# mstksg/tensor-ops

Hardware: AMD Instinct MI355X
Metric: gradTOp steps/sec (ffLayer MNIST 784->256->10) + gmul TFLOP/s vs roofline (higher is better)
Workload: dtype f32

## Files before the change

tensor-ops_amd/csrc/gemm_small.hip:

```cpp
#include "common.hpp"

#include <type_traits>

namespace to {

typedef float f32x16 __attribute__((ext_vector_type(16)));

template <class S>
struct SmallArgsT {
  const S* A;
  const S* B;
  S* C;
  const S* Cin;
  int M, N, K;
  long a_sm, a_sk, b_sk, b_sn, c_sm;
  long a_sb, b_sb, c_sb;
  int a_vec, b_vec;
  unsigned a_bytes, b_bytes;
  int tiles_n;
  int tiles_m;
  int tile_order;
  int kper;
  S alpha, beta;
  const S* bias;
// ... 17 lines not shown
};

#ifdef TOPS_AB_KNOBS
#define SM_STAMP(i) do { if (stamp_on) g.dbg[i] = wall_clock64(); } while (0)
#else
#define SM_STAMP(i) do { } while (0)
#endif


template <class G>
__device__ __forceinline__ void tile_of(const G& g, int bid, int& tile_m, int& tile_n) {
  if (g.tile_order) {
    const int T = g.tiles_m * g.tiles_n, x = bid & 7, q = T >> 3, r = T & 7;
    bid = (x < r ? x * (q + 1) : r * (q + 1) + (x - r) * q) + (bid >> 3);
  }
  if (g.tile_order == 2) {
    tile_n = bid / g.tiles_m;
    tile_m = bid - tile_n * g.tiles_m;
  } else {
    tile_m = bid / g.tiles_n;
    tile_n = bid - tile_m * g.tiles_n;
  }
}

__device__ __forceinline__ float tanh_s(float x) { return tanhf(x); }
__device__ __forceinline__ double tanh_s(double x) { return tanh(x); }
__device__ __forceinline__ float exp_s(float x) { return expf(x); }
__device__ __forceinline__ double exp_s(double x) { return exp(x); }
__device__ __forceinline__ float log_s(float x) { return logf(x); }
__device__ __forceinline__ double log_s(double x) { return log(x); }
__device__ __forceinline__ float max_s(float a, float b) { return fmaxf(a, b); }
__device__ __forceinline__ double max_s(double a, double b) { return fmax(a, b); }

template <class S, int AMODE, int BMODE, int NW, int TS, int ONESHOT = 0, bool EXT = false, int PARTS = 0, bool STAG = false>
__device__ __forceinline__ void gemm_small_body(const SmallArgsT<S>& g, const int bid, const long bz, S* ext_lds = nullptr,
                                                const int tid_in = -1) {
  constexpr int ES = (int)sizeof(S);
  static_assert(ES == 4 || TS == 16, "the fp64 matrix instruction is 16x16x4");
  constexpr int KG = (TS == 32) ? 2 : 4;
  constexpr int NR = (TS == 32) ? 16 : 4;
  constexpr int CK = 4 * KG;
  typedef S accv __attribute__((ext_vector_type(NR)));
  S (*red)[NR][64];
  S (*rsum)[64];
  S* dzs;
  if constexpr (EXT) {
    red = reinterpret_cast<S (*)[NR][64]>(ext_lds);
    rsum = reinterpret_cast<S (*)[64]>(ext_lds + NW * NR * 64);
    dzs = ext_lds + NW * NR * 64 + NW * 64;
  } else {
    __shared__ S red_s[NW][NR][64];
    __shared__ S rsum_s[NW][64];
    __shared__ S dzs_s[TS == 16 ? 16 * 17 : 1];
    red = red_s;
    rsum = rsum_s;
    dzs = dzs_s;
  }
  const int tid = tid_in >= 0 ? tid_in : (int)threadIdx.x, lane = tid & 63, wave = tid >> 6;
  const int l31 = lane & (TS - 1), half = lane / TS;
#ifdef TOPS_AB_KNOBS
  const bool stamp_on = g.dbg && bid == 0 && tid == 0;
#endif
  SM_STAMP(0);
  int tile_m, tile_n;
  tile_of(g, bid, tile_m, tile_n);
  const long m = (long)tile_m * TS + l31, n = (long)tile_n * TS + l31;
// ... 204 lines not shown
    }
  }
#pragma unroll
  for (int r = 0; r < NR; ++r) red[wave][r][lane] = acc[r];
  rsum[wave][lane] = asum;
  SM_STAMP(4);
  __syncthreads();
  SM_STAMP(5);
  if (g.rowsum && tile_n == 0 && wave == 0 && lane < TS) {
    S v = S(0);
#pragma unroll
    for (int w = 0; w < NW; ++w)
#pragma unroll
      for (int q = 0; q < KG; ++q) v += rsum[w][lane + q * TS];
    const long row = (long)tile_m * TS + lane;
    if (row < g.M) g.rowsum[bz * g.M + row] = g.rowsum_acc ? g.rowsum_in[bz * g.M + row] + g.rowsum_alpha * v : v;
  }
#pragma unroll
  for (int i = 0; i < NRW; ++i) {
    const int r = wave + i * NW;
    if (r >= NR) break;
    S v = S(0);
#pragma unroll
    for (int w = 0; w < NW; ++w) v += red[w][r][lane];
    const int lrow = (TS == 32) ? (r & 3) + 8 * (r >> 2) + 4 * half : row16(half, r);
    const long row = (long)tile_m * TS + lrow;
    const long col = (long)tile_n * TS + l31;
    if constexpr (TS == 16) {
      if (g.loss_rows) {
        const bool valid = row < g.M && col < g.N;
        v = v * g.alpha + pf_bias;
        const S t = valid ? g.target[row * g.c_sm + col] : S(0);
        auto sum16 = [](S x) {
#pragma unroll
          for (int off = 8; off > 0; off >>= 1) x += __shfl_xor(x, off, 64);
          return x;
        };
        S out, l;
        if (g.loss_rows == 1) {
          S mx = valid ? v : S(-INFINITY);
#pragma unroll
          for (int off = 8; off > 0; off >>= 1) mx = max_s(mx, __shfl_xor(mx, off, 64));
          const S e = valid ? exp_s(v - mx) : S(0);
          const S se = sum16(e), sy = sum16(t);
          const S pr = e / se;
          out = pr * sy - t;
          l = valid ? -t * log_s(pr) : S(0);
        } else {
          const S sg = S(1) / (S(1) + exp_s(-v));
          const S e = t - sg;
          out = S(-2) * e * sg * (S(1) - sg);
          l = valid ? e * e : S(0);
        }
        if (valid) Cb[row * g.c_sm + col] = out;
        if (g.tail_out) dzs[lrow * 17 + l31] = valid ? out : S(0);
        if (g.loss_out) {
          l = sum16(l);
          if (l31 == 0 && row < g.M) g.loss_out[row] = l;
        }
        continue;
      }
    }
    if (row < g.M && col < g.N) {
      v *= g.alpha;
      if (Ci) v += g.beta * pf_ci[i];
      v += pf_bias;
      if (g.act == 1) v = S(1) / (S(1) + exp_s(-v));
      else if (g.act == 2) v = tanh_s(v);
      if (Hd) {
        const S h = pf_hd[i];
        v *= g.dact_kind ? S(1) - h * h : h * (S(1) - h);
      }
      Cb[row * g.c_sm + col] = v;
    }
  }
// ... 12 lines not shown
#pragma unroll
      for (int st = 0; st < 4; ++st) {
        if (4 * st < g.N) {
          const S a = dzs[l15 * 17 + 4 * st + kg];
#pragma unroll
          for (int u = 0; u < 2; ++u) {
            if constexpr (ES == 8) acc2[u] = __builtin_amdgcn_mfma_f64_16x16x4f64(a, tl_bw[u][st], acc2[u], 0, 0, 0);
            else acc2[u] = __builtin_amdgcn_mfma_f32_16x16x4f32(a, tl_bw[u][st], acc2[u], 0, 0, 0);
          }
        }
      }
#pragma unroll
      for (int u = 0; u < 2; ++u) {
        const int t = wave + u * NW;
        const long col = (long)t * 16 + l15;
#pragma unroll
        for (int r = 0; r < 4; ++r) {
          const long row = (long)tile_m * 16 + row16(kg, r);
          if (t < ntiles && row < g.M && col < g.tail_n)
            g.tail_out[row * g.tail_n + col] = acc2[u][r] * tl_hv[u][r] * (S(1) - tl_hv[u][r]);
        }
      }
      SM_STAMP(7);
    }
  }
#ifdef TOPS_AB_KNOBS
  if (stamp_on) { __builtin_amdgcn_s_waitcnt(0); SM_STAMP(8); }
#endif
}

template <class S, int AMODE, int BMODE, int NW, int TS, int ONESHOT = 0>
__global__ __launch_bounds__(NW * 64) void gemm_small_kernel(SmallArgsT<S> g) {
  gemm_small_body<S, AMODE, BMODE, NW, TS, ONESHOT>(g, (int)blockIdx.x, (long)blockIdx.z);
}

template <class S, int A1, int B1, int NW1, int TS1, int OS1, int A2, int B2, int NW2, int TS2, int OS2, int P1 = 0, bool STAG1 = false>
__global__ __launch_bounds__((NW1 > NW2 ? NW1 : NW2) * 64) void gemm_small_pair_kernel(SmallArgsT<S> g1,
                                                                                         SmallArgsT<S> g2, int n1) {
  if ((int)blockIdx.x < n1) {
    if (NW1 < NW2 && (int)(threadIdx.x >> 6) >= NW1) return;
    gemm_small_body<S, A1, B1, NW1, TS1, OS1, false, P1, STAG1>(g1, (int)blockIdx.x, 0);
  } else {
    if (NW2 < NW1 && (int)(threadIdx.x >> 6) >= NW2) return;
    gemm_small_body<S, A2, B2, NW2, TS2, OS2>(g2, (int)blockIdx.x - n1, 0);
  }
}

struct ChainSync {
  unsigned* ctr;
  int* status;
  long long timeout;
  int dev;
};

__device__ __forceinline__ bool chain_barrier(const ChainSync& cs, int which, unsigned epoch) {
  __shared__ int ok;
  if (cs.dev == 1) {
    __syncthreads();
    return true;
  }
  if (cs.dev != 2) __builtin_amdgcn_fence(__ATOMIC_RELEASE, "agent");
  if (threadIdx.x == 0) ok = 1;
  __syncthreads();
  unsigned* flags = cs.ctr + which * 256;
  if (threadIdx.x == 0) __hip_atomic_store(flags + blockIdx.x, epoch, __ATOMIC_RELEASE, __HIP_MEMORY_SCOPE_AGENT);
  if (threadIdx.x < gridDim.x) {
// ... 433 lines not shown
}

template <class S>
static void launch_small_t(const GemmProblem& p, hipStream_t s) {
  constexpr bool F64 = sizeof(S) == 8;
  SmallArgsT<S> g;
  const SmallPlan c = plan_small<S>(p, g);
#ifdef TOPS_AB_KNOBS
  if (g.loss_rows) g.dbg = small_stamps(2);
#endif
  const int amode = c.amode, bmode = c.bmode;
  if constexpr (F64) {
    if (c.f64_t32) {
      const int tiles_m = (int)((p.M + 31) / 32);
      dim3 grid(tiles_m * g.tiles_n, 1, (unsigned)p.batch), block(c.nw * 64);
#define TOPS_F64_T32(AM, BM)                                                                              \
  switch (c.nw * 10 + c.os) {                                                                             \
    case 22: launch_k((gemm_small_f64_t32_kernel<AM, BM, 2, 2>), grid, block, 0, s, g); break;  \
    case 42: launch_k((gemm_small_f64_t32_kernel<AM, BM, 4, 2>), grid, block, 0, s, g); break;  \
    default: launch_k((gemm_small_f64_t32_kernel<AM, BM, 8, 1>), grid, block, 0, s, g); break;  \
  }
      switch (amode * 2 + bmode) {
        case 0: TOPS_F64_T32(0, 0) break;
        case 1: TOPS_F64_T32(0, 1) break;
        case 2: TOPS_F64_T32(1, 0) break;
        default: TOPS_F64_T32(1, 1) break;
      }
#undef TOPS_F64_T32
      TO_HIP(hipGetLastError());
      count_launch();
      return;
    }
  }
  if (c.os == 8 && c.nw == 16) {
    if constexpr (!F64) launch_nw<S, 16, 32, 8>(g, p, amode, bmode, s);
  } else if (c.os == 8) {
    launch_nw<S, 8, 16, 8>(g, p, amode, bmode, s);
  } else if (c.ts == 16) {
    switch (c.nw) {
      case 1: launch_nw<S, 1, 16>(g, p, amode, bmode, s); break;
      case 2: launch_nw<S, 2, 16>(g, p, amode, bmode, s); break;
      case 4: launch_nw<S, 4, 16>(g, p, amode, bmode, s); break;
      default: launch_nw<S, 8, 16>(g, p, amode, bmode, s); break;
    }
  } else {
    if constexpr (!F64) {
      switch (c.nw) {
        case 1: launch_nw<S, 1, 32>(g, p, amode, bmode, s); break;
        case 2: launch_nw<S, 2, 32>(g, p, amode, bmode, s); break;
        case 4: launch_nw<S, 4, 32>(g, p, amode, bmode, s); break;
        default: launch_nw<S, 8, 32>(g, p, amode, bmode, s); break;
      }
    }
  }
  TO_HIP(hipGetLastError());
  count_launch();
}

static int* g_chain_status = nullptr;

bool launch_gemm_small_chain(const GemmProblem& pa, const GemmProblem& pb, const GemmProblem& pc1, const GemmProblem& pc2,
                             hipStream_t s) {
  static const int enable = [] { const char* e = ab_getenv("TOPS_STEP_CHAIN"); return e ? atoi(e) : 0; }();
  if (!enable) return false;
  const GemmProblem* ps[4] = {&pa, &pb, &pc1, &pc2};
  for (const GemmProblem* p : ps)
    if (p->dtype != TO_F32 || p->batch != 1 || !gemm_small_can(*p)) return false;
// ... 146 lines not shown
    launch_gemm_t32(p, s);
    return;
  }
  if (p.dtype == TO_F64) launch_small_t<double>(p, s);
  else launch_small_t<float>(p, s);
}

constexpr int SMALL_PAIR_PARTS = 8;
constexpr bool SMALL_PAIR_STAG = false;

bool launch_gemm_small_pair(const GemmProblem& p1, const GemmProblem& p2, hipStream_t s) {
  static const int enable = [] { const char* e = ab_getenv("TOPS_SMALL_PAIR"); return e ? atoi(e) : 1; }();
  if (!enable || p1.dtype != p2.dtype || p1.batch != 1 || p2.batch != 1) return false;
  if (launch_gemm_t32_pair(p1, p2, s)) return true;
  if (!gemm_small_can(p1) || !gemm_small_can(p2)) return false;
  if (p1.dtype == TO_F64) {
    SmallArgsT<double> g1, g2;
    const SmallPlan c1 = plan_small<double>(p1, g1), c2 = plan_small<double>(p2, g2);
    if (!(c1.f64_t32 && c1.nw == 8 && c1.os == 1 && c1.amode == 1 && c1.bmode == 0)) return false;
    if (!(!c2.f64_t32 && c2.ts == 16 && c2.nw == 8 && c2.os == 8 && c2.amode == 1 && c2.bmode == 0)) return false;
    if (g1.loss_rows || g2.loss_rows) return false;
    const int n1 = (int)((p1.M + 31) / 32) * g1.tiles_n, n2 = (int)((p2.M + 15) / 16) * g2.tiles_n;
    launch_k((gemm_small_pair_f64_kernel<1, 0, 1, 0>), dim3(n1 + n2), dim3(512), 0, s, g1, g2, n1);
    TO_HIP(hipGetLastError());
    count_launch();
    return true;
  }
  SmallArgsT<float> g1, g2;
  const SmallPlan c1 = plan_small<float>(p1, g1), c2 = plan_small<float>(p2, g2);
#ifdef TOPS_AB_KNOBS
  g1.dbg = small_stamps(1);
  g2.dbg = small_stamps(3);
#endif
  if (!(c1.ts == 32 && c1.nw == 16 && c1.os == 8 && c1.amode == 1 && c1.bmode == 0)) return false;
  if (!(c2.ts == 16 && c2.nw == 8 && c2.os == 8 && c2.amode == 1 && c2.bmode == 0)) return false;
  if (g1.loss_rows || g2.loss_rows) return false;
  const int n1 = (int)((p1.M + 31) / 32) * g1.tiles_n, n2 = (int)((p2.M + 15) / 16) * g2.tiles_n;
  dim3 grid(n1 + n2), block(1024);
#define TOPS_PAIR(P, ST) launch_k((gemm_small_pair_kernel<float, 1, 0, 16, 32, 8, 1, 0, 8, 16, 8, P, ST>), grid, block, 0, s, g1, g2, n1)
#ifdef TOPS_AB_KNOBS
  static const int parts = [] { const char* e = ab_getenv("TOPS_SMALL_PARTS"); return e ? atoi(e) : SMALL_PAIR_PARTS; }();
  static const int stag = [] { const char* e = ab_getenv("TOPS_SMALL_STAGGER"); return e ? atoi(e) : (int)SMALL_PAIR_STAG; }();
  switch (parts * 2 + (stag ? 1 : 0)) {
    case 0: TOPS_PAIR(0, false); break;
    case 2: TOPS_PAIR(1, false); break;
    case 3: TOPS_PAIR(1, true); break;
    case 4: TOPS_PAIR(2, false); break;
    case 5: TOPS_PAIR(2, true); break;
    case 8: TOPS_PAIR(4, false); break;
    case 9: TOPS_PAIR(4, true); break;
    case 16: TOPS_PAIR(8, false); break;
    case 17: TOPS_PAIR(8, true); break;
    default: TO_CHECK(false, TO_ERR_ARG, "TOPS_SMALL_PARTS is 0, 1, 2, 4 or 8 (TOPS_SMALL_STAGGER needs parts >= 1)");
  }
#else
  TOPS_PAIR(SMALL_PAIR_PARTS, SMALL_PAIR_STAG);
#endif
#undef TOPS_PAIR
  TO_HIP(hipGetLastError());
  count_launch();
  return true;
}

}
```

tensor-ops_amd/csrc/gemm_t32.hip:

```cpp
#include <cstdio>
#include <type_traits>

#include "common.hpp"

namespace to {

typedef float f32x16 __attribute__((ext_vector_type(16)));
typedef float f32x4 __attribute__((ext_vector_type(4)));

struct T32Args {
  const float* A;
  const float* B;
  float* C;
  const float* Cin;
  const float* bias;
  const float* dact;
  float* rowsum;
  const float* rowsum_in;
  unsigned long long* dbg;
  long a_sx, b_sx;
  long c_sm;
  int M, N, K;
  int tiles_m, tiles_n;
  int gm, gn;
  int act, dact_kind;
  int rowsum_acc;
  int pd;
  float alpha, beta;
  float rowsum_alpha;
};

__device__ __attribute__((aligned(16))) float g_t32_zero[4] = {0.f, 0.f, 0.f, 0.f};

constexpr int T32_BK = 32, T32_NS = 2, T32_NW = 4;
constexpr int T32_CTR = 4096;
constexpr int T32_STAGE = 2 * 32 * T32_BK;
constexpr int T32_WAVE = T32_NS * T32_STAGE;

__device__ __forceinline__ bool t32_tile_of(int tiles_m, int tiles_n, int gm, int gn, int bid, int& tm, int& tn) {
  const int x = bid & 7, local = bid >> 3, xm = x / gn, xn = x - xm * gn;
  const int r0 = tiles_m * xm / gm, r1 = tiles_m * (xm + 1) / gm, c0 = tiles_n * xn / gn, c1 = tiles_n * (xn + 1) / gn;
  const int w = c1 - c0;
  if (w <= 0 || local >= (r1 - r0) * w) return false;
  tm = r0 + local / w;
  tn = c0 + local - (local / w) * w;
  return true;
}

__device__ __forceinline__ int t32_key(int x) { return (x >> 1) & 7; }

template <bool AKC, bool BKC, bool ARAG = false, bool WT = false, int NW = T32_NW, int NS = T32_NS, bool EARLY = false>
__device__ __forceinline__ int gemm_t32_body(const T32Args& g, const int bid, float* smem) {
  constexpr int WAVE_F = NS * T32_STAGE;
  static_assert(WAVE_F >= 1024 + 64, "a wave's stage memory holds its partial tile and its row sums");
  static_assert(!ARAG || !AKC, "the dword form is for a row-contiguous A");
  constexpr int NA = ARAG ? 16 : 4, PER = NA + 4;
  const int tid = threadIdx.x, lane = tid & 63;
  const int wave = __builtin_amdgcn_readfirstlane(tid >> 6);
  const int l31 = lane & 31, half = lane >> 5;
  unsigned long long* const dbg = (g.dbg && tid == 0 && (bid == 0 || bid == (int)gridDim.x - 1)) ? g.dbg + (bid == 0 ? 0 : 8) : nullptr;
  auto stamp = [&](int i) { if (dbg) dbg[i] = __builtin_amdgcn_s_memrealtime(); };
  int tile_m, tile_n;
  if (!t32_tile_of(g.tiles_m, g.tiles_n, g.gm, g.gn, bid, tile_m, tile_n)) return -1;
  stamp(0);
  const int m0 = tile_m * 32, n0 = tile_n * 32;

  const int erow = tid >> 3, ec4 = (tid & 7) * 4;
  const long grow = m0 + erow, gcol = n0 + ec4;
  const bool evalid = (NW == 4 || tid < 256) && grow < g.M && gcol < g.N;
  f32x4 pf_ci = {0.f, 0.f, 0.f, 0.f}, pf_hd = {0.f, 0.f, 0.f, 0.f}, pf_bias = {0.f, 0.f, 0.f, 0.f};
  auto prefetch_epilogue = [&] {
    if (evalid) {
      if (g.Cin) pf_ci = *reinterpret_cast<const f32x4*>(g.Cin + grow * g.c_sm + gcol);
      if (g.dact) pf_hd = *reinterpret_cast<const f32x4*>(g.dact + grow * g.c_sm + gcol);
      if (g.bias) pf_bias = *reinterpret_cast<const f32x4*>(g.bias + gcol);
    }
  };
  if constexpr (!EARLY) prefetch_epilogue();

  const int U = (g.K + 15) / 16;
  const int k0 = (int)((long)U * wave / NW) * 16;
  int k1 = (int)((long)U * (wave + 1) / NW) * 16;
  if (k1 > g.K) k1 = g.K;
  const int nC = k1 > k0 ? (k1 - k0 + T32_BK - 1) / T32_BK : 0;

  typedef __attribute__((address_space(3))) void* lptr_t;
  float* wsm = smem + wave * WAVE_F;
  const unsigned lds_w = __builtin_amdgcn_readfirstlane((unsigned)(unsigned long)(lptr_t)wsm);

  const int lr = lane >> 3, ls = lane & 7;
  unsigned oa[4], ob[4];
  bool xa_ok = true, xb_ok = true;
#pragma unroll
  for (int p = 0; p < 4; ++p) {
    if constexpr (AKC) {
      long x = m0 + 8 * p + lr;
      if (x >= g.M) x = g.M - 1;
      oa[p] = (unsigned)((x * g.a_sx + 4 * (ls ^ t32_key(8 * p + lr))) * 4);
    } else {
      oa[p] = (unsigned)(((long)(8 * p + lr) * g.a_sx + m0 + 4 * ls) * 4);
    }
    if constexpr (BKC) {
      long x = n0 + 8 * p + lr;
      if (x >= g.N) x = g.N - 1;
      ob[p] = (unsigned)((x * g.b_sx + 4 * (ls ^ t32_key(8 * p + lr))) * 4);
    } else {
      ob[p] = (unsigned)(((long)(8 * p + lr) * g.b_sx + n0 + 4 * ls) * 4);
    }
  }
  if constexpr (!AKC) xa_ok = m0 + 4 * ls + 3 < g.M;
  if constexpr (!BKC) xb_ok = n0 + 4 * ls + 3 < g.N;
  const bool interior = !ARAG && (AKC || m0 + 32 <= g.M) && (BKC || n0 + 32 <= g.N);
  const long step_a = AKC ? T32_BK * 4L : T32_BK * g.a_sx * 4L, step_b = BKC ? T32_BK * 4L : T32_BK * g.b_sx * 4L;
  const char* sa = reinterpret_cast<const char*>(g.A) + (AKC ? (long)k0 * 4 : (long)k0 * g.a_sx * 4);
  const char* sb = reinterpret_cast<const char*>(g.B) + (BKC ? (long)k0 * 4 : (long)k0 * g.b_sx * 4);

#define T32_DMA(OFF, BASE) asm volatile("global_load_lds_dwordx4 %0, %1 offset:0" ::"v"(OFF), "s"(BASE) : "memory")
#define T32_DMA_V(PTR) asm volatile("global_load_lds_dwordx4 %0, off offset:0" ::"v"(PTR) : "memory")
  const long a_sx_l = g.a_sx;
  const int M_l = g.M;
  auto issue = [&, a_sx_l, M_l](int c) {
    const int seq = c;
    const int kc = k0 + c * T32_BK;
    const unsigned st = lds_w + (unsigned)(seq % NS) * (T32_STAGE * 4);
    const char* ba = sa + (long)c * step_a;
    const char* bb = sb + (long)c * step_b;
    const bool full = kc + T32_BK <= k1;
    if (full && interior) {
#pragma unroll
      for (int p = 0; p < 4; ++p) {
        asm volatile("s_mov_b32 m0, %0\n\ts_nop 0" ::"s"(st + p * 1024) : "memory");
        T32_DMA(oa[p], ba);
      }
#pragma unroll
      for (int p = 0; p < 4; ++p) {
        asm volatile("s_mov_b32 m0, %0\n\ts_nop 0" ::"s"(st + 4096 + p * 1024) : "memory");
        T32_DMA(ob[p], bb);
      }
    } else {
      const char* zero = reinterpret_cast<const char*>(g_t32_zero);
      if constexpr (ARAG) {
#pragma unroll
        for (int e = 0; e < 16; ++e) {
          const int kl = 2 * e + half;
          const bool ok = kc + kl < k1 && m0 + l31 < M_l;
          const char* src = ok ? ba + ((long)kl * a_sx_l + m0 + l31) * 4 : zero;
          asm volatile("s_mov_b32 m0, %0\n\ts_nop 0" ::"s"(st + e * 256) : "memory");
          asm volatile("global_load_lds_dword %0, off offset:0" ::"v"(src) : "memory");
        }
      } else {
#pragma unroll
        for (int p = 0; p < 4; ++p) {
          const bool ok = AKC ? (kc + 4 * (ls ^ t32_key(8 * p + lr)) < k1) : (kc + 8 * p + lr < k1 && xa_ok);
          const char* src = ok ? ba + oa[p] : zero;
          asm volatile("s_mov_b32 m0, %0\n\ts_nop 0" ::"s"(st + p * 1024) : "memory");
          T32_DMA_V(src);
        }
      }
#pragma unroll
      for (int p = 0; p < 4; ++p) {
        const bool ok = BKC ? (kc + 4 * (ls ^ t32_key(8 * p + lr)) < k1) : (kc + 8 * p + lr < k1 && xb_ok);
        const char* src = ok ? bb + ob[p] : zero;
        asm volatile("s_mov_b32 m0, %0\n\ts_nop 0" ::"s"(st + 4096 + p * 1024) : "memory");
        T32_DMA_V(src);
      }
    }
  };
#undef T32_DMA
#undef T32_DMA_V

  f32x16 acc;
#pragma unroll
  for (int r = 0; r < 16; ++r) acc[r] = 0.f;
  float asum = 0.f;
  const bool want_rs = g.rowsum != nullptr && tile_n == 0;

  const int PD = g.pd < NS ? g.pd : NS;
  const int pro = nC < PD ? nC : PD;
  if constexpr (EARLY) {
    if (pro > 0) issue(0);
    __builtin_amdgcn_sched_barrier(0);
    prefetch_epilogue();
    __builtin_amdgcn_sched_barrier(0);
    for (int c = 1; c < pro; ++c) issue(c);
  } else {
    for (int c = 0; c < pro; ++c) issue(c);
  }
  stamp(1);

  auto wait_landed = [&](int c) {
    const int newer = (nC - 1 - c) < (PD - 1) ? (nC - 1 - c) : (PD - 1);
    static_assert(3 * PER <= 63, "vmcnt is six bits");
    if (newer >= 3) asm volatile("s_waitcnt vmcnt(%0)" ::"n"(3 * PER) : "memory");
    else if (newer == 2) asm volatile("s_waitcnt vmcnt(%0)" ::"n"(2 * PER) : "memory");
    else if (newer == 1) asm volatile("s_waitcnt vmcnt(%0)" ::"n"(PER) : "memory");
    else asm volatile("s_waitcnt vmcnt(0)" ::: "memory");
  };
  auto steps_of = [&](int c) { return (k1 - (k0 + c * T32_BK)) > 16 ? 4 : 2; };
  auto read_frags = [&](int c, float (&fa)[16], float (&fb)[16]) {
    const float* sp = wsm + (c % NS) * T32_STAGE;
    const int nI = steps_of(c);
#pragma unroll
    for (int i = 0; i < 4; ++i) {
      if (i < nI) {
        if constexpr (AKC) {
          const f32x4 v = *reinterpret_cast<const f32x4*>(sp + l31 * 32 + 4 * ((2 * i + half) ^ t32_key(l31)));
          fa[4 * i] = v.x; fa[4 * i + 1] = v.y; fa[4 * i + 2] = v.z; fa[4 * i + 3] = v.w;
        } else {
#pragma unroll
          for (int j = 0; j < 4; ++j) fa[4 * i + j] = sp[(4 * (2 * i + half) + j) * 32 + l31];
        }
        if constexpr (BKC) {
          const f32x4 v = *reinterpret_cast<const f32x4*>(sp + 1024 + l31 * 32 + 4 * ((2 * i + half) ^ t32_key(l31)));
          fb[4 * i] = v.x; fb[4 * i + 1] = v.y; fb[4 * i + 2] = v.z; fb[4 * i + 3] = v.w;
        } else {
#pragma unroll
          for (int j = 0; j < 4; ++j) fb[4 * i + j] = sp[1024 + (4 * (2 * i + half) + j) * 32 + l31];
        }
      }
    }
  };
  auto mma = [&](int c, const float (&fa)[16], const float (&fb)[16]) {
    const int nI = steps_of(c);
#pragma unroll
    for (int i = 0; i < 4; ++i) {
      if (i < nI) {
#pragma unroll
        for (int j = 0; j < 4; ++j) {
          acc = __builtin_amdgcn_mfma_f32_32x32x2f32(fa[4 * i + j], fb[4 * i + j], acc, 0, 0, 0);
          if (want_rs) asum += fa[4 * i + j];
        }
      }
    }
  };
  float fa[16], fb[16];
  for (int c = 0; c < nC; ++c) {
    wait_landed(c);
    if (c == 0) stamp(2);
    read_frags(c, fa, fb);
    asm volatile("s_waitcnt lgkmcnt(0)" ::: "memory");
    __builtin_amdgcn_sched_barrier(0);
    if (c + PD < nC) issue(c + PD);
    __builtin_amdgcn_sched_barrier(0);
    mma(c, fa, fb);
  }
  asm volatile("s_waitcnt vmcnt(0)" ::: "memory");
  stamp(3);

#pragma unroll
  for (int r = 0; r < 16; ++r) wsm[((r & 3) + 8 * (r >> 2) + 4 * half) * 32 + l31] = acc[r];
  if (want_rs) wsm[1024 + lane] = asum;
  __syncthreads();
  stamp(4);
  f32x4 s = {0.f, 0.f, 0.f, 0.f};
  if (NW == 4 || tid < 256) {
    s = *reinterpret_cast<const f32x4*>(smem + erow * 32 + ec4);
#pragma unroll
    for (int w = 1; w < NW; ++w) s += *reinterpret_cast<const f32x4*>(smem + w * WAVE_F + erow * 32 + ec4);
  }
  if (evalid) {
    f32x4 v = s * g.alpha;
    if (g.Cin) v += pf_ci * g.beta;
    if (g.bias) v += pf_bias;
    if (g.act == 1) {
      v.x = 1.f / (1.f + __expf(-v.x)); v.y = 1.f / (1.f + __expf(-v.y));
      v.z = 1.f / (1.f + __expf(-v.z)); v.w = 1.f / (1.f + __expf(-v.w));
    } else if (g.act == 2) {
      v.x = tanhf(v.x); v.y = tanhf(v.y); v.z = tanhf(v.z); v.w = tanhf(v.w);
    }
    if (g.dact) {
      if (g.dact_kind == 0) v *= pf_hd * (1.f - pf_hd);
      else v *= 1.f - pf_hd * pf_hd;
    }
    if constexpr (WT) {
      typedef unsigned int u32x4 __attribute__((ext_vector_type(4)));
      const u32x4 u = {__float_as_uint(v.x), __float_as_uint(v.y), __float_as_uint(v.z), __float_as_uint(v.w)};
      float* dst = g.C + grow * g.c_sm + gcol;
      asm volatile("global_store_dwordx4 %0, %1, off sc0 sc1" ::"v"(dst), "v"(u) : "memory");
    } else {
      *reinterpret_cast<f32x4*>(g.C + grow * g.c_sm + gcol) = v;
    }
  }
  if (want_rs && tid < 32) {
    const long m = m0 + tid;
    if (m < g.M) {
      float t = 0.f;
#pragma unroll
      for (int w = 0; w < NW; ++w) t += smem[w * WAVE_F + 1024 + tid] + smem[w * WAVE_F + 1024 + 32 + tid];
      if (g.rowsum_acc) g.rowsum[m] = (g.rowsum_in ? g.rowsum_in[m] : g.rowsum[m]) + g.rowsum_alpha * t;
      else g.rowsum[m] = t;
    }
  }
  stamp(5);
  return tile_m;
}

struct T32HeadArgs {
  const float* W2;
  const float* bias2;
  const float* target;
  float* dz;
  float* loss_out;
  float* tail_out;
  unsigned* ctr;
  int* status;
  long w_sn, dz_sm;
  int N2, loss_rows;
  float alpha2;
};

__global__ __launch_bounds__(256) void gemm_t32_head_kernel(T32Args g, T32HeadArgs h) {
  extern __shared__ __attribute__((aligned(1024))) float t32_smem[];
  const int tid = threadIdx.x, lane = tid & 63;
  const int wave = __builtin_amdgcn_readfirstlane(tid >> 6);
  const unsigned long long t_entry = g.dbg ? __builtin_amdgcn_s_memrealtime() : 0ull;
  int tile_m, tile_n;
  if (!t32_tile_of(g.tiles_m, g.tiles_n, g.gm, g.gn, (int)blockIdx.x, tile_m, tile_n)) return;
  const long grow = (long)tile_m * 32 + 4 * tile_n + wave;
  const bool rv = grow < g.M;
  f32x4 w4[16];
#pragma unroll
  for (int n = 0; n < 16; ++n) {
    w4[n] = f32x4{0.f, 0.f, 0.f, 0.f};
    if (n < h.N2) w4[n] = *reinterpret_cast<const f32x4*>(h.W2 + (long)n * h.w_sn + 4 * lane);
  }
  const float b_l = (lane < h.N2 && h.bias2) ? h.bias2[lane] : 0.f;
// ... 69 lines not shown
    out_l = lv ? -2.f * e * sg * (1.f - sg) : 0.f;
    loss_l = lv ? e * e : 0.f;
  }
  if (rv) {
    if (lv) h.dz[grow * h.dz_sm + lane] = out_l;
    if (h.loss_out) {
      const float l = sum16(loss_l);
      if (lane == 0) h.loss_out[grow] = l;
    }
  }
  if (hd) hd[3] = __builtin_amdgcn_s_memrealtime();
  if (h.tail_out) {
    f32x4 a = {0.f, 0.f, 0.f, 0.f};
#pragma unroll
    for (int n = 0; n < 16; ++n)
      if (n < h.N2) {
        const float d = __shfl(out_l, n, 64);
        a += w4[n] * d;
      }
    if (rv) *reinterpret_cast<f32x4*>(h.tail_out + grow * 256 + 4 * lane) = a * h4 * (1.f - h4);
  }
  if (hd) hd[4] = __builtin_amdgcn_s_memrealtime();
  __syncthreads();
  if (tid == 0) {
    unsigned* leave = h.ctr + T32_CTR + tile_m;
    const unsigned seen = __hip_atomic_fetch_add(leave, 1u, __ATOMIC_RELAXED, __HIP_MEMORY_SCOPE_AGENT);
    if (seen == (unsigned)(g.tiles_n - 1)) {
      __hip_atomic_store(h.ctr + tile_m, 0u, __ATOMIC_RELAXED, __HIP_MEMORY_SCOPE_AGENT);
      __hip_atomic_store(leave, 0u, __ATOMIC_RELAXED, __HIP_MEMORY_SCOPE_AGENT);
    }
  }
}

template <bool AKC, bool BKC, int NW = T32_NW, int NS = T32_NS, bool EARLY = false>
__global__ __launch_bounds__(NW * 64) void gemm_t32_kernel(T32Args g) {
  extern __shared__ __attribute__((aligned(1024))) float t32_smem[];
  gemm_t32_body<AKC, BKC, false, false, NW, NS, EARLY>(g, (int)blockIdx.x, t32_smem);
}

template <bool ARAG2>
__global__ __launch_bounds__(256) void gemm_t32_pair_kernel(T32Args g1, T32Args g2, int n1) {
  extern __shared__ __attribute__((aligned(1024))) float t32_smem[];
  if ((int)blockIdx.x < n1) gemm_t32_body<false, false, false>(g1, (int)blockIdx.x, t32_smem);
  else gemm_t32_body<false, false, ARAG2>(g2, (int)blockIdx.x - n1, t32_smem);
}

static bool t32_fill(const GemmProblem& p, T32Args& g, bool& akc, bool& bkc, bool allow_ragged_a = false, bool* ragged_a = nullptr) {
  if (p.dtype != TO_F32 || p.batch != 1 || p.reduce_batch) return false;
  if (p.loss_rows || p.tail_out || p.loss_out) return false;
  akc = p.a_sk == 1 && p.K > 1;
  bkc = p.b_sk == 1 && p.K > 1;
  if (!akc && p.a_sm != 1) return false;
  if (!bkc && p.b_sn != 1) return false;
  if (p.K % 4 != 0 || p.N % 4 != 0) return false;
  const bool rag = !akc && (p.M % 4 != 0 || p.a_sk % 4 != 0 || (reinterpret_cast<uintptr_t>(p.A) & 15u));
  if (ragged_a) *ragged_a = rag;
  if (rag && !allow_ragged_a) return false;
  if (akc && p.a_sm % 4 != 0) return false;
  if (bkc && p.b_sn % 4 != 0) return false;
  if (!bkc && p.b_sk % 4 != 0) return false;
  if ((reinterpret_cast<uintptr_t>(p.A) & 3u) || ((akc || !rag) && (reinterpret_cast<uintptr_t>(p.A) & 15u))) return false;
  if ((reinterpret_cast<uintptr_t>(p.B) | reinterpret_cast<uintptr_t>(p.C)) & 15u) return false;
  if (p.c_sm % 4 != 0) return false;
  if (p.Cin && (reinterpret_cast<uintptr_t>(p.Cin) & 15u)) return false;
  if (p.dact && (reinterpret_cast<uintptr_t>(p.dact) & 15u)) return false;
  if (p.bias && (reinterpret_cast<uintptr_t>(p.bias) & 15u)) return false;
  if (p.beta != 0.0 && !p.Cin) return false;
  if (p.act > 2) return false;
  if ((p.M + 32) * std::max<int64_t>(p.a_sm, 1) * 4 + p.K * std::max<int64_t>(p.a_sk, 1) * 4 >= (1LL << 31)) return false;
  if ((p.N + 32) * std::max<int64_t>(p.b_sn, 1) * 4 + p.K * std::max<int64_t>(p.b_sk, 1) * 4 >= (1LL << 31)) return false;
  g.A = (const float*)p.A; g.B = (const float*)p.B; g.C = (float*)p.C;
  g.Cin = p.beta != 0.0 ? (const float*)p.Cin : nullptr;
  g.M = (int)p.M; g.N = (int)p.N; g.K = (int)p.K;
  g.a_sx = akc ? p.a_sm : p.a_sk;
  g.b_sx = bkc ? p.b_sn : p.b_sk;
  g.c_sm = p.c_sm;
  g.tiles_m = (int)((p.M + 31) / 32); g.tiles_n = (int)((p.N + 31) / 32);
  {
    int best = 1 << 30;
    for (int gm : {8, 4, 2, 1}) {
      const int gn = 8 / gm;
      const int cost = (g.tiles_m + gm - 1) / gm + (g.tiles_n + gn - 1) / gn;
      if (cost < best) { best = cost; g.gm = gm; g.gn = gn; }
    }
  }
  g.alpha = (float)p.alpha; g.beta = (float)p.beta;
  g.bias = (const float*)p.bias; g.dact = (const float*)p.dact; g.act = p.act; g.dact_kind = p.dact_kind;
  g.rowsum = (float*)p.rowsum; g.rowsum_in = (const float*)p.rowsum_in; g.rowsum_alpha = (float)p.rowsum_alpha;
  g.rowsum_acc = p.rowsum_acc ? 1 : 0;
  static const int pd = [] { const char* e = ab_getenv("TOPS_T32_PD"); const int v = e ? atoi(e) : 2; return v < 1 ? 1 : (v > T32_NS ? T32_NS : v); }();
  g.pd = pd;
  static unsigned long long* dbg = [] {
    unsigned long long* p = nullptr;
    if (ab_getenv("TOPS_T32_STAMPS") && hipHostMalloc(reinterpret_cast<void**>(&p), 16 * sizeof(unsigned long long), hipHostMallocMapped) == hipSuccess) {
      for (int i = 0; i < 16; ++i) p[i] = 0;
      static unsigned long long* keep = p;
      atexit([] {
        if (keep[15]) {
          const unsigned long long* k = keep + 8;
          std::fprintf(stderr, "[t32] joined launch, workgroup 0, us since it began: its tile stored and arrived %.2f, all eight tiles of the row block "
                               "there %.2f, loss head of its four rows done %.2f, tail stored %.2f (entered %.2f us after stamp 0)\n",
                       (k[1] - k[0]) * 0.01, (k[2] - k[0]) * 0.01, (k[3] - k[0]) * 0.01, (k[4] - k[0]) * 0.01, ((double)k[0] - (double)keep[0]) * 0.01);
        }
        for (int w = 0; w < (keep[15] ? 1 : 2); ++w) {
          const unsigned long long* k = keep + 8 * w;
          std::fprintf(stderr, "[t32] %s workgroup of the last launch, us since it began: prologue DMA issued %.2f, first chunk landed %.2f, K loop done %.2f, "
                               "partials met %.2f, done %.2f; began %.2f us after workgroup 0\n", w ? "last" : "first",
                       (k[1] - k[0]) * 0.01, (k[2] - k[0]) * 0.01, (k[3] - k[0]) * 0.01, (k[4] - k[0]) * 0.01, (k[5] - k[0]) * 0.01,
                       ((double)k[0] - (double)keep[0]) * 0.01);
        }
      });
    }
    return p;
  }();
  g.dbg = dbg;
  return true;
}

bool gemm_t32_applicable(const GemmProblem& p) {
  static const int enable = [] { const char* e = ab_getenv("TOPS_GEMM_T32"); return e ? atoi(e) : 1; }();
  if (!enable) return false;
  T32Args g;
  bool akc, bkc;
  if (!t32_fill(p, g, akc, bkc)) return false;
  const long tiles = (long)g.tiles_m * g.tiles_n;
  static const long max_tiles = [] { const char* e = ab_getenv("TOPS_T32_MAXTILES"); return e ? atol(e) : 512L; }();
  return tiles >= 96 && tiles <= max_tiles && p.K >= 256 && p.K <= 8192;
}

bool launch_gemm_t32_pair(const GemmProblem& p1, const GemmProblem& p2, hipStream_t s);

static long t32_grid(const T32Args& g) {
  const long rm = (g.tiles_m + g.gm - 1) / g.gm, rn = (g.tiles_n + g.gn - 1) / g.gn;
  return 8 * rm * rn;
}

static void t32_attr(const void* k) { TO_HIP(hipFuncSetAttribute(k, hipFuncAttributeMaxDynamicSharedMemorySize, T32_NW * T32_WAVE * 4)); }

constexpr int T32_W8_DEFAULT = 1;
constexpr int T32_W8_NS = 1;
constexpr bool T32_EARLY = true;

template <int NW, int NS, bool EARLY>
static void t32_launch_nw(const T32Args& g, bool akc, bool bkc, hipStream_t s) {
  constexpr size_t lds = (size_t)NW * NS * T32_STAGE * 4;
  static bool attr = false;
  if (!attr) {
    TO_HIP(hipFuncSetAttribute(reinterpret_cast<const void*>(gemm_t32_kernel<true, true, NW, NS, EARLY>), hipFuncAttributeMaxDynamicSharedMemorySize, (int)lds));
    TO_HIP(hipFuncSetAttribute(reinterpret_cast<const void*>(gemm_t32_kernel<true, false, NW, NS, EARLY>), hipFuncAttributeMaxDynamicSharedMemorySize, (int)lds));
    TO_HIP(hipFuncSetAttribute(reinterpret_cast<const void*>(gemm_t32_kernel<false, true, NW, NS, EARLY>), hipFuncAttributeMaxDynamicSharedMemorySize, (int)lds));
    TO_HIP(hipFuncSetAttribute(reinterpret_cast<const void*>(gemm_t32_kernel<false, false, NW, NS, EARLY>), hipFuncAttributeMaxDynamicSharedMemorySize, (int)lds));
    attr = true;
  }
  const dim3 grid((unsigned)t32_grid(g)), block(NW * 64);
  if (akc && bkc) launch_k((gemm_t32_kernel<true, true, NW, NS, EARLY>), grid, block, lds, s, g);
  else if (akc) launch_k((gemm_t32_kernel<true, false, NW, NS, EARLY>), grid, block, lds, s, g);
  else if (bkc) launch_k((gemm_t32_kernel<false, true, NW, NS, EARLY>), grid, block, lds, s, g);
  else launch_k((gemm_t32_kernel<false, false, NW, NS, EARLY>), grid, block, lds, s, g);
}

void launch_gemm_t32(const GemmProblem& p, hipStream_t s) {
  T32Args g;
  bool akc, bkc;
  TO_CHECK(t32_fill(p, g, akc, bkc), TO_ERR_STATE, "launch_gemm_t32: not applicable");
  static const int cus = [] { hipDeviceProp_t pr; int d = 0; return (hipGetDevice(&d) == hipSuccess && hipGetDeviceProperties(&pr, d) == hipSuccess) ? pr.multiProcessorCount : 0; }();
  static const int waves = [] { const char* e = ab_getenv("TOPS_T32_WAVES"); return e ? atoi(e) : (T32_W8_DEFAULT ? 8 : 4); }();
  const bool w8 = waves == 8 && t32_grid(g) <= cus;
#ifdef TOPS_AB_KNOBS
  static const int w8_ns = [] { const char* e = ab_getenv("TOPS_T32_W8_NS"); return e ? atoi(e) : T32_W8_NS; }();
  static const int early = [] { const char* e = ab_getenv("TOPS_T32_EARLY"); return e ? atoi(e) : (int)T32_EARLY; }();
  switch ((w8 ? (w8_ns == 1 ? 2 : 4) : 0) + (early ? 1 : 0)) {
    case 0: t32_launch_nw<T32_NW, T32_NS, false>(g, akc, bkc, s); break;
    case 1: t32_launch_nw<T32_NW, T32_NS, true>(g, akc, bkc, s); break;
    case 2: t32_launch_nw<8, 1, false>(g, akc, bkc, s); break;
    case 3: t32_launch_nw<8, 1, true>(g, akc, bkc, s); break;
    case 4: t32_launch_nw<8, 2, false>(g, akc, bkc, s); break;
    default: t32_launch_nw<8, 2, true>(g, akc, bkc, s); break;
  }
#else
  if (w8) t32_launch_nw<8, T32_W8_NS, T32_EARLY>(g, akc, bkc, s);
  else t32_launch_nw<T32_NW, T32_NS, T32_EARLY>(g, akc, bkc, s);
#endif
  TO_HIP(hipGetLastError());
  count_launch();
}

static unsigned* g_t32_ctr = nullptr;
static int *g_t32_status = nullptr, *g_t32_status_dev = nullptr;
static bool g_t32_head_off = false;
void gemm_t32_init() {
  if (g_t32_ctr) return;
  if (hipMalloc(&g_t32_ctr, 2 * T32_CTR * sizeof(unsigned)) != hipSuccess || hipMemset(g_t32_ctr, 0, 2 * T32_CTR * sizeof(unsigned)) != hipSuccess) {
    (void)hipGetLastError();
    g_t32_ctr = nullptr;
    return;
  }
  if (hipHostMalloc(&g_t32_status, sizeof(int), hipHostMallocMapped) == hipSuccess) {
    *g_t32_status = 0;
    if (hipHostGetDevicePointer(reinterpret_cast<void**>(&g_t32_status_dev), g_t32_status, 0) != hipSuccess) g_t32_status_dev = nullptr;
  }
  (void)hipGetLastError();
}
int gemm_t32_take_failure() {
  const int st = g_t32_status ? *g_t32_status : 0;
  if (st) {
    g_t32_head_off = true;
    *g_t32_status = 0;
    if (g_t32_ctr) (void)hipMemset(g_t32_ctr, 0, 2 * T32_CTR * sizeof(unsigned));
  }
  return st;
}

bool launch_gemm_t32_head(const GemmProblem& pf, const GemmProblem& ph, hipStream_t s) {
// ... 70 lines not shown
```

Baseline: 41930.

## Add DPP row reductions, lean loss-head kernel, one-wave pair fusion, register K-unit

The 16-lane reductions in the loss epilogue now use DPP lane permutes instead of generic shuffles. A dedicated loss-head kernel is specialised for 8 waves with one-shot mode 2 and vector loads, and is selected by default for small-K loss problems. A new pair path fuses two single-wave 16x16 GEMMs into one launch. In the t32 kernel, the eight-wave, one-stage form can load an odd trailing 16-wide K unit straight into registers and feed it to MFMA while the LDS DMA of the first chunk is in flight, which shortens each wave's LDS-fed loop. Per-wave timestamp probes are also added. Together these bring more code paths and inline-asm register handling, and so more correctness risk.

```diff
diff --git a/tensor-ops_amd/csrc/gemm_small.hip b/tensor-ops_amd/csrc/gemm_small.hip
--- a/tensor-ops_amd/csrc/gemm_small.hip
+++ b/tensor-ops_amd/csrc/gemm_small.hip
@@ -73,6 +73,21 @@
 __device__ __forceinline__ float max_s(float a, float b) { return fmaxf(a, b); }
 __device__ __forceinline__ double max_s(double a, double b) { return fmax(a, b); }
 
+template <int OFF>
+__device__ __forceinline__ float xor16(float x) {
+  const int v = __float_as_int(x);
+  if constexpr (OFF == 1) return __int_as_float(__builtin_amdgcn_update_dpp(v, v, 0xB1, 0xF, 0xF, false));
+  else if constexpr (OFF == 2) return __int_as_float(__builtin_amdgcn_update_dpp(v, v, 0x4E, 0xF, 0xF, false));
+  else if constexpr (OFF == 8) return __int_as_float(__builtin_amdgcn_update_dpp(v, v, 0x128, 0xF, 0xF, false));
+  else {
+    static_assert(OFF == 4, "xor 8, 4, 2 or 1");
+    const int up = __builtin_amdgcn_update_dpp(v, v, 0x104, 0xF, 0x5, false);
+    return __int_as_float(__builtin_amdgcn_update_dpp(up, v, 0x114, 0xF, 0xA, false));
+  }
+}
+template <int OFF>
+__device__ __forceinline__ double xor16(double x) { return __shfl_xor(x, OFF, 64); }
+
 template <class S, int AMODE, int BMODE, int NW, int TS, int ONESHOT = 0, bool EXT = false, int PARTS = 0, bool STAG = false>
 __device__ __forceinline__ void gemm_small_body(const SmallArgsT<S>& g, const int bid, const long bz, S* ext_lds = nullptr,
                                                 const int tid_in = -1) {
@@ -343,15 +358,14 @@
         v = v * g.alpha + pf_bias;
         const S t = valid ? g.target[row * g.c_sm + col] : S(0);
         auto sum16 = [](S x) {
-#pragma unroll
-          for (int off = 8; off > 0; off >>= 1) x += __shfl_xor(x, off, 64);
+          x += xor16<8>(x); x += xor16<4>(x); x += xor16<2>(x); x += xor16<1>(x);
           return x;
         };
         S out, l;
         if (g.loss_rows == 1) {
           S mx = valid ? v : S(-INFINITY);
-#pragma unroll
-          for (int off = 8; off > 0; off >>= 1) mx = max_s(mx, __shfl_xor(mx, off, 64));
+          mx = max_s(mx, xor16<8>(mx)); mx = max_s(mx, xor16<4>(mx));
+          mx = max_s(mx, xor16<2>(mx)); mx = max_s(mx, xor16<1>(mx));
           const S e = valid ? exp_s(v - mx) : S(0);
           const S se = sum16(e), sy = sum16(t);
           const S pr = e / se;
@@ -430,6 +444,12 @@
 template <class S, int AMODE, int BMODE, int NW, int TS, int ONESHOT = 0>
 __global__ __launch_bounds__(NW * 64) void gemm_small_kernel(SmallArgsT<S> g) {
   gemm_small_body<S, AMODE, BMODE, NW, TS, ONESHOT>(g, (int)blockIdx.x, (long)blockIdx.z);
+}
+
+__global__ __launch_bounds__(8 * 64) void gemm_small_head_kernel(SmallArgsT<float> g) {
+  g.a_vec = 1;
+  g.b_vec = 1;
+  gemm_small_body<float, 0, 1, 8, 16, 2>(g, (int)blockIdx.x, (long)blockIdx.z);
 }
 
 template <class S, int A1, int B1, int NW1, int TS1, int OS1, int A2, int B2, int NW2, int TS2, int OS2, int P1 = 0, bool STAG1 = false>
@@ -929,7 +949,17 @@
       return;
     }
   }
-  if (c.os == 8 && c.nw == 16) {
+  static const int head_lean = [] { const char* e = ab_getenv("TOPS_SMALL_HEAD_LEAN"); return e ? atoi(e) : 1; }();
+  bool lean = false;
+  if constexpr (!F64)
+    lean = head_lean && g.loss_rows && c.ts == 16 && c.nw == 8 && c.os == 0 && amode == 0 && bmode == 1 && g.a_vec && g.b_vec &&
+           p.K <= 8 * 2 * 16;
+  if (lean) {
+    if constexpr (!F64) {
+      const dim3 grid((unsigned)(g.tiles_m * g.tiles_n), 1, (unsigned)p.batch), block(8 * 64);
+      launch_k(gemm_small_head_kernel, grid, block, 0, s, g);
+    }
+  } else if (c.os == 8 && c.nw == 16) {
     if constexpr (!F64) launch_nw<S, 16, 32, 8>(g, p, amode, bmode, s);
   } else if (c.os == 8) {
     launch_nw<S, 8, 16, 8>(g, p, amode, bmode, s);
@@ -1142,6 +1172,15 @@
   g1.dbg = small_stamps(1);
   g2.dbg = small_stamps(3);
 #endif
+  if (c1.ts == 16 && c1.nw == 1 && c1.os == 0 && c1.amode == 1 && c1.bmode == 0 && !c1.f64_t32 &&
+      c2.ts == 16 && c2.nw == 1 && c2.os == 0 && c2.amode == 1 && c2.bmode == 0 && !c2.f64_t32 && !g1.loss_rows && !g2.loss_rows) {
+    const long t1 = (long)g1.tiles_m * g1.tiles_n, t2 = (long)g2.tiles_m * g2.tiles_n;
+    if (t1 + t2 > 65535) return false;
+    launch_k((gemm_small_pair_kernel<float, 1, 0, 1, 16, 0, 1, 0, 1, 16, 0>), dim3((unsigned)(t1 + t2)), dim3(64), 0, s, g1, g2, (int)t1);
+    TO_HIP(hipGetLastError());
+    count_launch();
+    return true;
+  }
   if (!(c1.ts == 32 && c1.nw == 16 && c1.os == 8 && c1.amode == 1 && c1.bmode == 0)) return false;
   if (!(c2.ts == 16 && c2.nw == 8 && c2.os == 8 && c2.amode == 1 && c2.bmode == 0)) return false;
   if (g1.loss_rows || g2.loss_rows) return false;
diff --git a/tensor-ops_amd/csrc/gemm_t32.hip b/tensor-ops_amd/csrc/gemm_t32.hip
--- a/tensor-ops_amd/csrc/gemm_t32.hip
+++ b/tensor-ops_amd/csrc/gemm_t32.hip
@@ -49,8 +49,9 @@
 
 __device__ __forceinline__ int t32_key(int x) { return (x >> 1) & 7; }
 
-template <bool AKC, bool BKC, bool ARAG = false, bool WT = false, int NW = T32_NW, int NS = T32_NS, bool EARLY = false>
+template <bool AKC, bool BKC, bool ARAG = false, bool WT = false, int NW = T32_NW, int NS = T32_NS, bool EARLY = false, bool REGU = false>
 __device__ __forceinline__ int gemm_t32_body(const T32Args& g, const int bid, float* smem) {
+  static_assert(!REGU || (NW == 8 && NS == 1 && EARLY && !ARAG), "the register unit belongs to the eight-wave, one-stage, early-DMA form");
   constexpr int WAVE_F = NS * T32_STAGE;
   static_assert(WAVE_F >= 1024 + 64, "a wave's stage memory holds its partial tile and its row sums");
   static_assert(!ARAG || !AKC, "the dword form is for a row-contiguous A");
@@ -60,6 +61,12 @@
   const int l31 = lane & 31, half = lane >> 5;
   unsigned long long* const dbg = (g.dbg && tid == 0 && (bid == 0 || bid == (int)gridDim.x - 1)) ? g.dbg + (bid == 0 ? 0 : 8) : nullptr;
   auto stamp = [&](int i) { if (dbg) dbg[i] = __builtin_amdgcn_s_memrealtime(); };
+#ifdef TOPS_AB_KNOBS
+  unsigned long long* const wdbg = (g.dbg && lane == 0 && wave < 8 && (bid == 0 || bid == (int)gridDim.x - 1)) ? g.dbg + 16 + (bid == 0 ? 0 : 16) + 2 * wave : nullptr;
+#define T32_WSTAMP(i) do { if (wdbg) wdbg[i] = __builtin_amdgcn_s_memrealtime(); } while (0)
+#else
+#define T32_WSTAMP(i) do { } while (0)
+#endif
   int tile_m, tile_n;
   if (!t32_tile_of(g.tiles_m, g.tiles_n, g.gm, g.gn, bid, tile_m, tile_n)) return -1;
   stamp(0);
@@ -82,7 +89,14 @@
   const int k0 = (int)((long)U * wave / NW) * 16;
   int k1 = (int)((long)U * (wave + 1) / NW) * 16;
   if (k1 > g.K) k1 = g.K;
-  const int nC = k1 > k0 ? (k1 - k0 + T32_BK - 1) / T32_BK : 0;
+  int kd = k1;
+  bool ru = false;
+  if constexpr (REGU) {
+    const int nU = (k1 - k0 + 15) / 16;
+    ru = (nU & 1) != 0;
+    if (ru) kd = k0 + (nU - 1) * 16;
+  }
+  const int nC = kd > k0 ? (kd - k0 + T32_BK - 1) / T32_BK : 0;
 
   typedef __attribute__((address_space(3))) void* lptr_t;
   float* wsm = smem + wave * WAVE_F;
@@ -125,7 +139,7 @@
     const unsigned st = lds_w + (unsigned)(seq % NS) * (T32_STAGE * 4);
     const char* ba = sa + (long)c * step_a;
     const char* bb = sb + (long)c * step_b;
-    const bool full = kc + T32_BK <= k1;
+    const bool full = kc + T32_BK <= kd;
     if (full && interior) {
 #pragma unroll
       for (int p = 0; p < 4; ++p) {
@@ -143,7 +157,7 @@
 #pragma unroll
         for (int e = 0; e < 16; ++e) {
           const int kl = 2 * e + half;
-          const bool ok = kc + kl < k1 && m0 + l31 < M_l;
+          const bool ok = kc + kl < kd && m0 + l31 < M_l;
           const char* src = ok ? ba + ((long)kl * a_sx_l + m0 + l31) * 4 : zero;
           asm volatile("s_mov_b32 m0, %0\n\ts_nop 0" ::"s"(st + e * 256) : "memory");
           asm volatile("global_load_lds_dword %0, off offset:0" ::"v"(src) : "memory");
@@ -151,7 +165,7 @@
       } else {
 #pragma unroll
         for (int p = 0; p < 4; ++p) {
-          const bool ok = AKC ? (kc + 4 * (ls ^ t32_key(8 * p + lr)) < k1) : (kc + 8 * p + lr < k1 && xa_ok);
+          const bool ok = AKC ? (kc + 4 * (ls ^ t32_key(8 * p + lr)) < kd) : (kc + 8 * p + lr < kd && xa_ok);
           const char* src = ok ? ba + oa[p] : zero;
           asm volatile("s_mov_b32 m0, %0\n\ts_nop 0" ::"s"(st + p * 1024) : "memory");
           T32_DMA_V(src);
@@ -159,7 +173,7 @@
       }
 #pragma unroll
       for (int p = 0; p < 4; ++p) {
-        const bool ok = BKC ? (kc + 4 * (ls ^ t32_key(8 * p + lr)) < k1) : (kc + 8 * p + lr < k1 && xb_ok);
+        const bool ok = BKC ? (kc + 4 * (ls ^ t32_key(8 * p + lr)) < kd) : (kc + 8 * p + lr < kd && xb_ok);
         const char* src = ok ? bb + ob[p] : zero;
         asm volatile("s_mov_b32 m0, %0\n\ts_nop 0" ::"s"(st + 4096 + p * 1024) : "memory");
         T32_DMA_V(src);
@@ -177,9 +191,77 @@
 
   const int PD = g.pd < NS ? g.pd : NS;
   const int pro = nC < PD ? nC : PD;
+  f32x4 ua4[2], ub4[2];
+  float ua1[8], ub1[8];
+  if constexpr (REGU) {
+    if (ru) {
+      const float* zero = g_t32_zero;
+#pragma unroll
+      for (int i = 0; i < 2; ++i) {
+        const int kq = kd + 4 * (2 * i + half);
+        if constexpr (AKC) {
+          long x = m0 + l31;
+          if (x >= g.M) x = g.M - 1;
+          const float* src = kq < k1 ? g.A + x * g.a_sx + kq : zero;
+          asm volatile("global_load_dwordx4 %0, %1, off" : "=&v"(ua4[i]) : "v"(src) : "memory");
+        } else {
+#pragma unroll
+          for (int j = 0; j < 4; ++j) {
+            const float* src = (kq + j < k1 && m0 + l31 < g.M) ? g.A + (long)(kq + j) * g.a_sx + m0 + l31 : zero;
+            asm volatile("global_load_dword %0, %1, off" : "=&v"(ua1[4 * i + j]) : "v"(src) : "memory");
+          }
+        }
+        if constexpr (BKC) {
+          long x = n0 + l31;
+          if (x >= g.N) x = g.N - 1;
+          const float* src = kq < k1 ? g.B + x * g.b_sx + kq : zero;
+          asm volatile("global_load_dwordx4 %0, %1, off" : "=&v"(ub4[i]) : "v"(src) : "memory");
+        } else {
+#pragma unroll
+          for (int j = 0; j < 4; ++j) {
+            const float* src = (kq + j < k1 && n0 + l31 < g.N) ? g.B + (long)(kq + j) * g.b_sx + n0 + l31 : zero;
+            asm volatile("global_load_dword %0, %1, off" : "=&v"(ub1[4 * i + j]) : "v"(src) : "memory");
+          }
+        }
+      }
+    }
+    __builtin_amdgcn_sched_barrier(0);
+  }
   if constexpr (EARLY) {
     if (pro > 0) issue(0);
     __builtin_amdgcn_sched_barrier(0);
+    if constexpr (REGU) {
+      if (ru) {
+        if (pro > 0) asm volatile("s_waitcnt vmcnt(%0)" ::"n"(PER) : "memory");
+        else asm volatile("s_waitcnt vmcnt(0)" ::: "memory");
+        float fu[8], gu[8];
+        if constexpr (AKC) {
+          asm volatile("" : "+v"(ua4[0]), "+v"(ua4[1]) :: "memory");
+#pragma unroll
+          for (int i = 0; i < 2; ++i) { fu[4 * i] = ua4[i].x; fu[4 * i + 1] = ua4[i].y; fu[4 * i + 2] = ua4[i].z; fu[4 * i + 3] = ua4[i].w; }
+        } else {
+          asm volatile("" : "+v"(ua1[0]), "+v"(ua1[1]), "+v"(ua1[2]), "+v"(ua1[3]), "+v"(ua1[4]), "+v"(ua1[5]), "+v"(ua1[6]), "+v"(ua1[7]) :: "memory");
+#pragma unroll
+          for (int q = 0; q < 8; ++q) fu[q] = ua1[q];
+        }
+        if constexpr (BKC) {
+          asm volatile("" : "+v"(ub4[0]), "+v"(ub4[1]) :: "memory");
+#pragma unroll
+          for (int i = 0; i < 2; ++i) { gu[4 * i] = ub4[i].x; gu[4 * i + 1] = ub4[i].y; gu[4 * i + 2] = ub4[i].z; gu[4 * i + 3] = ub4[i].w; }
+        } else {
+          asm volatile("" : "+v"(ub1[0]), "+v"(ub1[1]), "+v"(ub1[2]), "+v"(ub1[3]), "+v"(ub1[4]), "+v"(ub1[5]), "+v"(ub1[6]), "+v"(ub1[7]) :: "memory");
+#pragma unroll
+          for (int q = 0; q < 8; ++q) gu[q] = ub1[q];
+        }
+        __builtin_amdgcn_sched_barrier(0);
+#pragma unroll
+        for (int q = 0; q < 8; ++q) {
+          acc = __builtin_amdgcn_mfma_f32_32x32x2f32(fu[q], gu[q], acc, 0, 0, 0);
+          if (want_rs) asum += fu[q];
+        }
+      }
+      __builtin_amdgcn_sched_barrier(0);
+    }
     prefetch_epilogue();
     __builtin_amdgcn_sched_barrier(0);
     for (int c = 1; c < pro; ++c) issue(c);
@@ -196,7 +278,7 @@
     else if (newer == 1) asm volatile("s_waitcnt vmcnt(%0)" ::"n"(PER) : "memory");
     else asm volatile("s_waitcnt vmcnt(0)" ::: "memory");
   };
-  auto steps_of = [&](int c) { return (k1 - (k0 + c * T32_BK)) > 16 ? 4 : 2; };
+  auto steps_of = [&](int c) { return (kd - (k0 + c * T32_BK)) > 16 ? 4 : 2; };
   auto read_frags = [&](int c, float (&fa)[16], float (&fb)[16]) {
     const float* sp = wsm + (c % NS) * T32_STAGE;
     const int nI = steps_of(c);
@@ -246,10 +328,12 @@
   }
   asm volatile("s_waitcnt vmcnt(0)" ::: "memory");
   stamp(3);
+  T32_WSTAMP(0);
 
 #pragma unroll
   for (int r = 0; r < 16; ++r) wsm[((r & 3) + 8 * (r >> 2) + 4 * half) * 32 + l31] = acc[r];
   if (want_rs) wsm[1024 + lane] = asum;
+  T32_WSTAMP(1);
   __syncthreads();
   stamp(4);
   f32x4 s = {0.f, 0.f, 0.f, 0.f};
@@ -292,6 +376,7 @@
     }
   }
   stamp(5);
+#undef T32_WSTAMP
   return tile_m;
 }
 
@@ -427,10 +512,10 @@
   }
 }
 
-template <bool AKC, bool BKC, int NW = T32_NW, int NS = T32_NS, bool EARLY = false>
+template <bool AKC, bool BKC, int NW = T32_NW, int NS = T32_NS, bool EARLY = false, bool REGU = false>
 __global__ __launch_bounds__(NW * 64) void gemm_t32_kernel(T32Args g) {
   extern __shared__ __attribute__((aligned(1024))) float t32_smem[];
-  gemm_t32_body<AKC, BKC, false, false, NW, NS, EARLY>(g, (int)blockIdx.x, t32_smem);
+  gemm_t32_body<AKC, BKC, false, false, NW, NS, EARLY, REGU>(g, (int)blockIdx.x, t32_smem);
 }
 
 template <bool ARAG2>
@@ -487,8 +572,8 @@
   g.pd = pd;
   static unsigned long long* dbg = [] {
     unsigned long long* p = nullptr;
-    if (ab_getenv("TOPS_T32_STAMPS") && hipHostMalloc(reinterpret_cast<void**>(&p), 16 * sizeof(unsigned long long), hipHostMallocMapped) == hipSuccess) {
-      for (int i = 0; i < 16; ++i) p[i] = 0;
+    if (ab_getenv("TOPS_T32_STAMPS") && hipHostMalloc(reinterpret_cast<void**>(&p), 48 * sizeof(unsigned long long), hipHostMallocMapped) == hipSuccess) {
+      for (int i = 0; i < 48; ++i) p[i] = 0;
       static unsigned long long* keep = p;
       atexit([] {
         if (keep[15]) {
@@ -503,6 +588,11 @@
                                "partials met %.2f, done %.2f; began %.2f us after workgroup 0\n", w ? "last" : "first",
                        (k[1] - k[0]) * 0.01, (k[2] - k[0]) * 0.01, (k[3] - k[0]) * 0.01, (k[4] - k[0]) * 0.01, (k[5] - k[0]) * 0.01,
                        ((double)k[0] - (double)keep[0]) * 0.01);
+          const unsigned long long* wv = keep + 16 + 16 * w;
+          std::fprintf(stderr, "[t32]   per wave, K loop done / partial written:");
+          for (int q = 0; q < 8; ++q)
+            if (wv[2 * q]) std::fprintf(stderr, "  w%d %.2f / %.2f", q, ((double)wv[2 * q] - (double)k[0]) * 0.01, ((double)wv[2 * q + 1] - (double)k[0]) * 0.01);
+          std::fprintf(stderr, "\n");
         }
       });
     }
@@ -535,23 +625,24 @@
 constexpr int T32_W8_DEFAULT = 1;
 constexpr int T32_W8_NS = 1;
 constexpr bool T32_EARLY = true;
-
-template <int NW, int NS, bool EARLY>
+constexpr bool T32_REGU = true;
+
+template <int NW, int NS, bool EARLY, bool REGU = false>
 static void t32_launch_nw(const T32Args& g, bool akc, bool bkc, hipStream_t s) {
   constexpr size_t lds = (size_t)NW * NS * T32_STAGE * 4;
   static bool attr = false;
   if (!attr) {
-    TO_HIP(hipFuncSetAttribute(reinterpret_cast<const void*>(gemm_t32_kernel<true, true, NW, NS, EARLY>), hipFuncAttributeMaxDynamicSharedMemorySize, (int)lds));
-    TO_HIP(hipFuncSetAttribute(reinterpret_cast<const void*>(gemm_t32_kernel<true, false, NW, NS, EARLY>), hipFuncAttributeMaxDynamicSharedMemorySize, (int)lds));
-    TO_HIP(hipFuncSetAttribute(reinterpret_cast<const void*>(gemm_t32_kernel<false, true, NW, NS, EARLY>), hipFuncAttributeMaxDynamicSharedMemorySize, (int)lds));
-    TO_HIP(hipFuncSetAttribute(reinterpret_cast<const void*>(gemm_t32_kernel<false, false, NW, NS, EARLY>), hipFuncAttributeMaxDynamicSharedMemorySize, (int)lds));
+    TO_HIP(hipFuncSetAttribute(reinterpret_cast<const void*>(gemm_t32_kernel<true, true, NW, NS, EARLY, REGU>), hipFuncAttributeMaxDynamicSharedMemorySize, (int)lds));
+    TO_HIP(hipFuncSetAttribute(reinterpret_cast<const void*>(gemm_t32_kernel<true, false, NW, NS, EARLY, REGU>), hipFuncAttributeMaxDynamicSharedMemorySize, (int)lds));
+    TO_HIP(hipFuncSetAttribute(reinterpret_cast<const void*>(gemm_t32_kernel<false, true, NW, NS, EARLY, REGU>), hipFuncAttributeMaxDynamicSharedMemorySize, (int)lds));
+    TO_HIP(hipFuncSetAttribute(reinterpret_cast<const void*>(gemm_t32_kernel<false, false, NW, NS, EARLY, REGU>), hipFuncAttributeMaxDynamicSharedMemorySize, (int)lds));
     attr = true;
   }
   const dim3 grid((unsigned)t32_grid(g)), block(NW * 64);
-  if (akc && bkc) launch_k((gemm_t32_kernel<true, true, NW, NS, EARLY>), grid, block, lds, s, g);
-  else if (akc) launch_k((gemm_t32_kernel<true, false, NW, NS, EARLY>), grid, block, lds, s, g);
-  else if (bkc) launch_k((gemm_t32_kernel<false, true, NW, NS, EARLY>), grid, block, lds, s, g);
-  else launch_k((gemm_t32_kernel<false, false, NW, NS, EARLY>), grid, block, lds, s, g);
+  if (akc && bkc) launch_k((gemm_t32_kernel<true, true, NW, NS, EARLY, REGU>), grid, block, lds, s, g);
+  else if (akc) launch_k((gemm_t32_kernel<true, false, NW, NS, EARLY, REGU>), grid, block, lds, s, g);
+  else if (bkc) launch_k((gemm_t32_kernel<false, true, NW, NS, EARLY, REGU>), grid, block, lds, s, g);
+  else launch_k((gemm_t32_kernel<false, false, NW, NS, EARLY, REGU>), grid, block, lds, s, g);
 }
 
 void launch_gemm_t32(const GemmProblem& p, hipStream_t s) {
@@ -564,16 +655,20 @@
 #ifdef TOPS_AB_KNOBS
   static const int w8_ns = [] { const char* e = ab_getenv("TOPS_T32_W8_NS"); return e ? atoi(e) : T32_W8_NS; }();
   static const int early = [] { const char* e = ab_getenv("TOPS_T32_EARLY"); return e ? atoi(e) : (int)T32_EARLY; }();
+  static const int regu = [] { const char* e = ab_getenv("TOPS_T32_REGU"); return e ? atoi(e) : (int)T32_REGU; }();
   switch ((w8 ? (w8_ns == 1 ? 2 : 4) : 0) + (early ? 1 : 0)) {
     case 0: t32_launch_nw<T32_NW, T32_NS, false>(g, akc, bkc, s); break;
     case 1: t32_launch_nw<T32_NW, T32_NS, true>(g, akc, bkc, s); break;
     case 2: t32_launch_nw<8, 1, false>(g, akc, bkc, s); break;
-    case 3: t32_launch_nw<8, 1, true>(g, akc, bkc, s); break;
+    case 3:
+      if (regu) t32_launch_nw<8, 1, true, true>(g, akc, bkc, s);
+      else t32_launch_nw<8, 1, true, false>(g, akc, bkc, s);
+      break;
     case 4: t32_launch_nw<8, 2, false>(g, akc, bkc, s); break;
     default: t32_launch_nw<8, 2, true>(g, akc, bkc, s); break;
   }
 #else
-  if (w8) t32_launch_nw<8, T32_W8_NS, T32_EARLY>(g, akc, bkc, s);
+  if (w8) t32_launch_nw<8, T32_W8_NS, T32_EARLY, T32_REGU>(g, akc, bkc, s);
   else t32_launch_nw<T32_NW, T32_NS, T32_EARLY>(g, akc, bkc, s);
 #endif
   TO_HIP(hipGetLastError());
```

Result: faster. 44240, median of 6 (+5.5%).
